# XieResearchGroup/Physics-aware-Multiplex-GNN

Measured on AMD Instinct MI355X. Metric: molecules/sec (QM9 dim=128 n_layer=6) at 1/2/4/8 GPU; scatter-add HBM GB/s vs peak, higher is better.
Workload: dtype f32; 1 GPU; QM9-schema synthetic radius-graph batches, PAMNet dim=128 n_layer=6, 128 molecules/GPU (BASELINE configs[1]), full training step fwd+bwd+allreduce+clip+Adam+EMA; global_batch=128, parallelism=dp1 (molecule-sharded, RCCL all-reduce of flat grad), nodes_per_batch=2286, global_edges=32888, local_edges=4316, triplets=6662, pairs=10978

## Files before the change

include/pamnet_hip.h:

```cpp
#ifndef PAMNET_HIP_H
#define PAMNET_HIP_H

#include <stdint.h>

#ifdef __cplusplus
extern "C" {
#endif

#define PAMNET_OK 0
#define PAMNET_EINVAL (-1)
#define PAMNET_ENULL (-2)
#define PAMNET_WEIGHT_IMAGES 2
#define PAMNET_CHAIN_PIECES 16

typedef void* pamnet_stream_t;

#define PAMNET_ABI_VERSION 18
int pamnet_abi_version(void);

int pamnet_segment_sum_f32(float* out, const float* init, const float* A, const int32_t* ia, const float* B,
                           const int32_t* ib, const int32_t* perm, const int32_t* ptr, int64_t rows, int64_t d,
                           pamnet_stream_t stream);

int pamnet_gather_mul_f32(float* out, const float* A, const int32_t* ia, const float* B, const int32_t* ib,
// ... 269 lines not shown
                         const int32_t* band_status, const uint8_t* climb, const double* k_b, double k, float* dneb,
                         double* seg, double* fpar, pamnet_stream_t stream);

int pamnet_vib_displace_f32(const float* pos0, const int32_t* gptr, const int32_t* fptr, const int32_t* free_idx, int64_t n,
                            int64_t n_graphs, int64_t pairs, int64_t t, double delta, float* pos_out, pamnet_stream_t stream);
int pamnet_vib_rows_f64(const float* dpos, const float* pos0, const float* masses, const int32_t* fptr, const int32_t* free_idx,
                        const int64_t* moff, int64_t n, int64_t n_graphs, int64_t pairs, int64_t t, double delta, double* h,
                        pamnet_stream_t stream);
int pamnet_sym_eig_f64(double* a, double* v, double* w, int32_t* status, int32_t* sweeps, const int64_t* moff,
                       const int64_t* dptr, int64_t n_mat, double tol, int32_t max_sweeps, pamnet_stream_t stream);

int pamnet_md_step_f32(float* pos, float* vel, const float* dpos, const float* mass, const uint8_t* fixed, const int32_t* gptr,
                       int64_t n, int64_t n_graphs, const int64_t* seed, int32_t* steps, int32_t* status, double* ke,
                       const double* dt_g, const double* kT_g, const double* gamma_g, double dt, double kT, double gamma,
                       int32_t kick_in, int32_t advance, pamnet_stream_t stream);
int pamnet_md_init_velocities_f32(float* vel, const float* mass, const uint8_t* fixed, const int32_t* gptr, int64_t n,
                                  int64_t n_graphs, const int64_t* seed, const double* kT_g, double kT, int32_t remove_com,
                                  int32_t rescale, double* ke, pamnet_stream_t stream);

int pamnet_md_npt_step_f32(float* pos, float* vel, const float* dpos, const float* dstrain, const float* mass,
                           const uint8_t* fixed, const int32_t* gptr, int64_t n, int64_t n_graphs, const float* cell0,
                           float* cell, double* eps, const uint8_t* cell_dof, const int64_t* seed, int32_t* steps,
                           int32_t* status, double* ke, double* pint, double* vol, const double* dt_g, const double* kT_g,
                           const double* gamma_g, const double* pressure_g, const double* rate_g, double dt, double kT,
                           double gamma, double pressure, double rate, int32_t kick_in, int32_t advance,
                           pamnet_stream_t stream);

int pamnet_fuse_pool_fwd_f32(const float* outs, const float* atts, int64_t n_layer, int64_t n, const float* sign,
                             const int32_t* gptr, int64_t n_graphs, int32_t mean, float* node_out, float* graph_out,
                             pamnet_stream_t stream);
int pamnet_fuse_pool_bwd_f32(const float* outs, const float* atts, int64_t n_layer, int64_t n, const float* sign,
                             const int32_t* node_graph, const int32_t* gptr, int32_t mean, const float* grad_graph,
                             float* grad_outs, float* grad_atts, pamnet_stream_t stream);

int pamnet_node_tail_fwd_f32(const float* x2, const float* res_x, int64_t n, const float* const* weights,
                             const float* const* biases, const float* w_out, const float* b_out, const float* w_att,
                             float* Z, float* R, float* x_out, float* out, float* att, const float* next_Wx1,
                             const float* next_bx1, const float* const* next_wp, int64_t next_ldwp, int64_t next_nblk,
                             float* next_Zx1, float* next_x1, float* next_P, int32_t packed, pamnet_stream_t stream);
int pamnet_node_tail_fwd_rider_f32(const float* x2, const float* res_x, int64_t n, const float* const* weights,
                                   const float* const* biases, const float* w_out, const float* b_out,
                                   const float* w_att, float* Z, float* R, float* x_out, const float* next_Wx1,
                                   const float* next_bx1, const float* const* next_wp, int64_t next_ldwp,
                                   int64_t next_nblk, float* next_Zx1, float* next_x1, float* next_P, const float* mlp_x,
                                   int64_t mlp_rows, int64_t mlp_tile0, int64_t mlp_ntiles, const float* const* mlp,
                                   float* const* mlp_out, int64_t rider_wgs, int32_t packed ,
                                   pamnet_stream_t stream);
int pamnet_node_heads_fwd_f32(int64_t n_layers, const float* const* x_out, const float* const* weights,
                              const float* const* biases, const float* const* w_out, const float* const* b_out,
                              const float* const* w_att, float* const* Z, float* const* out, float* const* att, int64_t n,
                              int32_t packed, pamnet_stream_t stream);
int pamnet_node_tail_bwd_f32(const float* d_xout, const float* d_out, const float* d_att, int64_t n,
                             const float* const* weights, const float* w_out, const float* w_att, const float* Z,
                             float* dZ, float* d_x2, float* d_resx, float* head_partial, float* d_wout, float* d_watt,
                             float* d_bout, int32_t packed, pamnet_stream_t stream);
int pamnet_node_heads_bwd_f32(int64_t n_layers, const float* const* d_out, const float* const* d_att,
                              const float* const* weights, const float* const* w_out, const float* const* w_att,
                              const float* const* Z, float* const* dZ3, float* const* g_head, float* const* head_partial,
                              int64_t n, int32_t packed, pamnet_stream_t stream);
int pamnet_node_tail_main_bwd_f32(const float* d_xout, const float* g_head, int64_t n, const float* const* weights,
                                  const float* Z, float* dZ, float* d_x2, float* d_resx, int32_t packed,
                                  pamnet_stream_t stream);
int pamnet_node_pre_tail_bwd_f32(const float* dP, const float* dx1_direct, const float* d_add, int64_t n,
                                 const float* Wx1, const float* const* wp, int64_t nblk, const float* Zx1, float* dZx1,
                                 const float* g_head, const float* const* weights, const float* Z, float* dZ,
                                 float* d_x2, float* d_resx, const void* rider ,
// ... 259 lines not shown
```

physics-aware-multiplex-gnn_amd/csrc/basis.hip:

```cpp
#include "common.h"
#include "basis_constants.h"

namespace {

__device__ __forceinline__ float envelope_f(float x) {
    if (!(x < 1.0f)) return 0.0f;
    const float x2 = x * x, x5 = x2 * x2 * x;
    return 1.0f / x + x5 * (-21.0f + x * (35.0f - 15.0f * x));
}

__device__ __forceinline__ double envelope_d(double x) {
    if (!(x < 1.0)) return 0.0;
    const double x2 = x * x, x5 = x2 * x2 * x;
    return 1.0 / x + x5 * (-21.0 + x * (35.0 - 15.0 * x));
}

constexpr int SERIES_TERMS = 28;
struct SeriesTab {
    double c[7][SERIES_TERMS + 1];
    double inv_dfact[7];
};
constexpr SeriesTab make_series() {
    SeriesTab t{};
    for (int l = 0; l < 7; ++l) {
        t.c[l][0] = 1.0;
        for (int k = 1; k <= SERIES_TERMS; ++k) t.c[l][k] = t.c[l][k - 1] * -0.5 / ((double)k * (double)(2 * l + 2 * k + 1));
        double d = 1.0;
        for (int m = 1; m <= l; ++m) d *= (double)(2 * m + 1);
        t.inv_dfact[l] = 1.0 / d;
    }
    return t;
}
__device__ __constant__ SeriesTab SBF_SERIES = make_series();
// ... 312 lines not shown
    const int lane = threadIdx.x & 63;
    if (q >= m) return;
    const double x = (double)(dist[q] * inv_cf);
    if (!(x < 1.0)) {
        if (lane == 0) ddist[q] = 0.0f;
        return;
    }
    double v = 0.0;
    if (lane < 42) {
        const int l = lane / 6;
        double acc = 0.0;
        for (int k = tt_ptr[q]; k < tt_ptr[q + 1]; ++k) {
            const int64_t t = tt_perm[k];
            const double ct = cos((double)angle[t]);
            double p0 = 1.0, p1 = ct;
            for (int j = 2; j <= l; ++j) {
                const double pj = ((double)(2 * j - 1) * ct * p1 - (double)(j - 1) * p0) / (double)j;
                p0 = p1;
                p1 = pj;
            }
            acc += (double)gsbf[t * 42 + lane] * PAMNET_YL0_PREF[l] * (l == 0 ? 1.0 : p1);
        }
        const double env = envelope_d(x), denv = envelope_dx_d(x);
        const double z = (double)PAMNET_SBF_ZEROS_F32[lane], u = z * x;
        const double jl = sph_jl(l, u);
        const double djl = (l == 0) ? -sph_jl(1, u) : sph_jl(l - 1, u) - (double)(l + 1) / u * jl;
        v = acc * PAMNET_SBF_NORM[lane] * (denv * jl + env * z * djl);
    }
#pragma unroll
    for (int o = 32; o >= 1; o >>= 1) v += __shfl_xor(v, o, 64);
    if (lane == 0) ddist[q] = (float)(v * inv_cutoff);
}

__device__ __forceinline__ float leaky02(float a) { return a > 0.f ? a : 0.2f * a; }

__global__ __launch_bounds__(256) void fuse_node_kernel(const float* __restrict__ outs, const float* __restrict__ atts,
                                                        int n_layer, int64_t n, const float* __restrict__ sign,
                                                        float* __restrict__ node_out) {
    const int64_t v = (int64_t)blockIdx.x * blockDim.x + threadIdx.x;
    if (v >= n) return;
    float acc = 0.f;
    for (int l = 0; l < n_layer; ++l) {
        const float ag = leaky02(atts[(int64_t)(2 * l) * n + v]), al = leaky02(atts[(int64_t)(2 * l + 1) * n + v]);
        const float mx = fmaxf(ag, al);
        const float eg = expf(ag - mx), el = expf(al - mx);
        const float inv = 1.0f / (eg + el);
        acc += (outs[(int64_t)(2 * l) * n + v] * eg + outs[(int64_t)(2 * l + 1) * n + v] * el) * inv;
    }
    node_out[v] = sign ? acc * sign[v] : acc;
}

__global__ __launch_bounds__(256) void pool_kernel(const float* __restrict__ node_out, const int32_t* __restrict__ gptr,
                                                   int64_t n_graphs, int mean, float* __restrict__ graph_out) {
    const int lane = threadIdx.x & 63;
    const int64_t g = ((int64_t)blockIdx.x * blockDim.x + threadIdx.x) >> 6;
    if (g >= n_graphs) return;
    const int beg = gptr[g], end = gptr[g + 1];
    float s0 = 0.f, s1 = 0.f, s2 = 0.f, s3 = 0.f;
    int v = beg + lane;
    for (; v + 192 < end; v += 256) {
        s0 += node_out[v];
        s1 += node_out[v + 64];
        s2 += node_out[v + 128];
        s3 += node_out[v + 192];
    }
    for (; v < end; v += 64) s0 += node_out[v];
    float s = (s0 + s1) + (s2 + s3);
#pragma unroll
    for (int o = 32; o >= 1; o >>= 1) s += __shfl_xor(s, o, 64);
    if (lane == 0) graph_out[g] = mean ? s / (float)max(end - beg, 1) : s;
}

__global__ __launch_bounds__(256) void fuse_pool_bwd_kernel(const float* __restrict__ outs,
                                                            const float* __restrict__ atts, int n_layer, int64_t n,
                                                            const float* __restrict__ sign,
                                                            const int32_t* __restrict__ node_graph,
                                                            const int32_t* __restrict__ gptr, int mean,
                                                            const float* __restrict__ grad_graph,
                                                            float* __restrict__ grad_outs,
                                                            float* __restrict__ grad_atts) {
    const int64_t v = (int64_t)blockIdx.x * blockDim.x + threadIdx.x;
    if (v >= n) return;
    const int g = node_graph[v];
    float gn = grad_graph[g];
    if (mean) gn /= (float)max(gptr[g + 1] - gptr[g], 1);
    if (sign) gn *= sign[v];
    for (int l = 0; l < n_layer; ++l) {
        const int64_t ig = (int64_t)(2 * l) * n + v, il = (int64_t)(2 * l + 1) * n + v;
        const float rg = atts[ig], rl = atts[il];
        const float ag = leaky02(rg), al = leaky02(rl);
        const float mx = fmaxf(ag, al);
        const float eg = expf(ag - mx), el = expf(al - mx);
        const float inv = 1.0f / (eg + el);
        const float wg = eg * inv, wl = el * inv;
        grad_outs[ig] = gn * wg;
        grad_outs[il] = gn * wl;
        const float da = gn * (outs[ig] - outs[il]) * wg * wl;
        grad_atts[ig] = da * (rg > 0.f ? 1.0f : 0.2f);
        grad_atts[il] = -da * (rl > 0.f ? 1.0f : 0.2f);
    }
}

inline unsigned blocks_for(int64_t n, int per = 256) { return (unsigned)(n > 0 ? ceil_div(n, per) : 1); }

}

extern "C" int pamnet_abi_version(void) { return PAMNET_ABI_VERSION; }

extern "C" int pamnet_rbf_fwd_f32(const float* dist, const float* freq, float cutoff, int64_t m, float* rbf,
                                  pamnet_stream_t stream) {
    if (m < 0 || !(cutoff > 0.f)) return PAMNET_EINVAL;
    if (m == 0) return PAMNET_OK;
    if (!dist || !freq || !rbf) return PAMNET_ENULL;
    hipLaunchKernelGGL(rbf_fwd_kernel, dim3(blocks_for(m * 16)), dim3(256), 0, as_stream(stream), dist, freq,
                       1.0f / cutoff, m, rbf);
    PAMNET_LAUNCH_CHECK();
    return PAMNET_OK;
}

extern "C" int pamnet_rbf_bwd_f32(const float* dist, const float* freq, float cutoff, int64_t m, const float* grad,
                                  float* dfreq, float* partial, pamnet_stream_t stream) {
    if (m < 0 || !(cutoff > 0.f)) return PAMNET_EINVAL;
    if (!dfreq || !partial || (m > 0 && (!dist || !freq || !grad))) return PAMNET_ENULL;
    hipStream_t st = as_stream(stream);
    int nblocks = (int)(m > 0 ? (ceil_div(m, 16) < 2048 ? ceil_div(m, 16) : 2048) : 0);
    if (nblocks > 0) {
        hipLaunchKernelGGL(rbf_bwd_partial_kernel, dim3(nblocks), dim3(256), 0, st, dist, freq, 1.0f / cutoff, m, grad,
                           partial);
        PAMNET_LAUNCH_CHECK();
    }
    hipLaunchKernelGGL(rbf_bwd_final_kernel, dim3(1), dim3(1024), 0, st, partial, nblocks, dfreq);
    PAMNET_LAUNCH_CHECK();
    return PAMNET_OK;
// ... 110 lines not shown

extern "C" int pamnet_fuse_pool_fwd_f32(const float* outs, const float* atts, int64_t n_layer, int64_t n,
                                        const float* sign, const int32_t* gptr, int64_t n_graphs, int32_t mean,
                                        float* node_out, float* graph_out, pamnet_stream_t stream) {
    if (n_layer <= 0 || n < 0 || n_graphs < 0) return PAMNET_EINVAL;
    if (n_graphs == 0) return PAMNET_OK;
    hipStream_t st = as_stream(stream);
    if (n == 0) {
        if (!graph_out) return PAMNET_ENULL;
        return (int)hipMemsetAsync(graph_out, 0, sizeof(float) * (size_t)n_graphs, st);
    }
    if (!outs || !atts || !gptr || !node_out || !graph_out) return PAMNET_ENULL;
    hipLaunchKernelGGL(fuse_node_kernel, dim3(blocks_for(n)), dim3(256), 0, st, outs, atts, (int)n_layer, n, sign,
                       node_out);
    PAMNET_LAUNCH_CHECK();
    hipLaunchKernelGGL(pool_kernel, dim3(blocks_for(n_graphs, 4)), dim3(256), 0, st, node_out, gptr, n_graphs,
                       (int)mean, graph_out);
    PAMNET_LAUNCH_CHECK();
    return PAMNET_OK;
}

extern "C" int pamnet_fuse_pool_bwd_f32(const float* outs, const float* atts, int64_t n_layer, int64_t n,
                                        const float* sign, const int32_t* node_graph, const int32_t* gptr,
                                        int32_t mean, const float* grad_graph, float* grad_outs, float* grad_atts,
                                        pamnet_stream_t stream) {
    if (n_layer <= 0 || n < 0) return PAMNET_EINVAL;
    if (n == 0) return PAMNET_OK;
    if (!outs || !atts || !node_graph || !gptr || !grad_graph || !grad_outs || !grad_atts) return PAMNET_ENULL;
    hipLaunchKernelGGL(fuse_pool_bwd_kernel, dim3(blocks_for(n)), dim3(256), 0, as_stream(stream), outs, atts,
                       (int)n_layer, n, sign, node_graph, gptr, (int)mean, grad_graph, grad_outs, grad_atts);
    PAMNET_LAUNCH_CHECK();
    return PAMNET_OK;
}
```

physics-aware-multiplex-gnn_amd/csrc/reduce.hip:

```cpp
#include "common.h"
#include "type_rows_core.h"

namespace {

constexpr int NORM_BLOCKS = 256;

__global__ __launch_bounds__(256) void sumsq_partials_kernel(const float4* __restrict__ g, int64_t n4,
                                                             double* __restrict__ partial) {
    __shared__ double red[256];
    float4 a0 = make_float4(0.f, 0.f, 0.f, 0.f), a1 = a0;
    const int64_t per = (n4 + gridDim.x - 1) / gridDim.x;
    const int64_t beg = blockIdx.x * per, end = beg + per < n4 ? beg + per : n4;
    int64_t i = beg + threadIdx.x;
    for (; i + 256 < end; i += 512) {
        const float4 u = g[i], v = g[i + 256];
        a0.x = fmaf(u.x, u.x, a0.x), a0.y = fmaf(u.y, u.y, a0.y), a0.z = fmaf(u.z, u.z, a0.z), a0.w = fmaf(u.w, u.w, a0.w);
        a1.x = fmaf(v.x, v.x, a1.x), a1.y = fmaf(v.y, v.y, a1.y), a1.z = fmaf(v.z, v.z, a1.z), a1.w = fmaf(v.w, v.w, a1.w);
    }
    if (i < end) {
        const float4 u = g[i];
        a0.x = fmaf(u.x, u.x, a0.x), a0.y = fmaf(u.y, u.y, a0.y), a0.z = fmaf(u.z, u.z, a0.z), a0.w = fmaf(u.w, u.w, a0.w);
    }
    red[threadIdx.x] = ((double)a0.x + (double)a0.y) + ((double)a0.z + (double)a0.w) + ((double)a1.x + (double)a1.y) +
                       ((double)a1.z + (double)a1.w);
    __syncthreads();
    for (int s = 128; s > 0; s >>= 1) {
        if ((int)threadIdx.x < s) red[threadIdx.x] += red[threadIdx.x + s];
        __syncthreads();
    }
    if (threadIdx.x == 0) partial[blockIdx.x] = red[0];
}

__global__ __launch_bounds__(256) void sumsq_partials_masked_kernel(const float4* __restrict__ g, int64_t n4,
// ... 22 lines not shown
    __syncthreads();
    for (int s = 128; s > 0; s >>= 1) {
        if ((int)threadIdx.x < s) red[threadIdx.x] += red[threadIdx.x + s];
        __syncthreads();
    }
    if (threadIdx.x == 0) partial[blockIdx.x] = red[0];
}

__global__ __launch_bounds__(256) void grad_accumulate_kernel(float4* __restrict__ acc, float4* __restrict__ g, int64_t n4) {
    const float4 zero = make_float4(0.f, 0.f, 0.f, 0.f);
    const int64_t stride = (int64_t)gridDim.x * 256;
    int64_t i = (int64_t)blockIdx.x * 256 + threadIdx.x;
    for (; i + stride < n4; i += 2 * stride) {
        float4 a0 = acc[i], a1 = acc[i + stride];
        const float4 g0 = g[i], g1 = g[i + stride];
        a0.x += g0.x, a0.y += g0.y, a0.z += g0.z, a0.w += g0.w;
        a1.x += g1.x, a1.y += g1.y, a1.z += g1.z, a1.w += g1.w;
        acc[i] = a0, acc[i + stride] = a1;
        g[i] = zero, g[i + stride] = zero;
    }
    if (i < n4) {
        float4 a0 = acc[i];
        const float4 g0 = g[i];
        a0.x += g0.x, a0.y += g0.y, a0.z += g0.z, a0.w += g0.w;
        acc[i] = a0;
        g[i] = zero;
    }
}

template <int KIND>
__global__ __launch_bounds__(256) void loss_kernel(const float* __restrict__ out, const float* __restrict__ y, int64_t n,
                                                   float grad_scale, float* __restrict__ loss, float* __restrict__ d_out) {
    __shared__ double red[256];
    double s = 0.0;
    const float gs = grad_scale / (float)n;
    for (int64_t i = threadIdx.x; i < n; i += 256) {
        const float d = out[i] - y[i];
        const float a = fabsf(d);
        float l, dl;
        if (KIND == 0) {
            l = a, dl = d > 0.f ? 1.f : (d < 0.f ? -1.f : 0.f);
        } else if (KIND == 1) {
            l = d * d, dl = 2.f * d;
        } else {
            l = a < 1.f ? 0.5f * d * d : a - 0.5f, dl = a < 1.f ? d : (d > 0.f ? 1.f : -1.f);
        }
        s += (double)l;
        if (d_out) d_out[i] = dl * gs;
    }
    red[threadIdx.x] = s;
    __syncthreads();
    for (int k = 128; k > 0; k >>= 1) {
        if ((int)threadIdx.x < k) red[threadIdx.x] += red[threadIdx.x + k];
        __syncthreads();
    }
    if (threadIdx.x == 0) loss[0] = (float)(red[0] / (double)n);
}

template <int KIND>
int loss_launch(const float* out, const float* y, int64_t n, float grad_scale, float* loss, float* d_out,
                pamnet_stream_t stream) {
    if (n < 1) return PAMNET_EINVAL;
    if (!out || !y || !loss) return PAMNET_ENULL;
    hipLaunchKernelGGL(loss_kernel<KIND>, dim3(1), dim3(256), 0, as_stream(stream), out, y, n, grad_scale, loss, d_out);
    PAMNET_LAUNCH_CHECK();
    return PAMNET_OK;
}

using type_rows::TYPE_BLOCKS;
using type_rows::TYPE_MAX;

__global__ __launch_bounds__(256) void type_rows_grad_kernel(const float4* __restrict__ g, const int32_t* __restrict__ idx,
                                                             int64_t n, int n_types, int d4, float4* __restrict__ partial) {
    __shared__ float4 red[256];
    type_rows::grad_body(g, idx, n, n_types, d4, partial, blockIdx.x, gridDim.x, red);
}

__global__ __launch_bounds__(256) void type_rows_finish_kernel(const float4* __restrict__ partial, int blocks, int cells,
                                                               float4* __restrict__ out) {
    type_rows::finish_body(partial, blocks, cells, out);
}

__global__ __launch_bounds__(256) void type_rows_grad_wide_kernel(const float4* __restrict__ g, const int32_t* __restrict__ idx,
                                                                  int64_t n, int n_types, int d4, uint32_t* __restrict__ masks,
                                                                  float4* __restrict__ partial) {
    __shared__ float4 red[256];
    __shared__ uint32_t seen[4];
    type_rows::grad_wide_body(g, idx, n, n_types, d4, masks, partial, blockIdx.x, gridDim.x, red, seen);
// ... 142 lines not shown
```

physics-aware-multiplex-gnn_amd/models.py:

```python
import math
import os

import torch
import torch.nn as nn
import torch.nn.functional as F

from pamnet_amd import fused, narrow, stack
from pamnet_amd import graph as G
from pamnet_amd import ops
from pamnet_amd.modules import MLP, BesselBasis, GlobalMP, LocalMP, mlp_apply


class Config(object):
    def __init__(self, dataset, dim, n_layer, cutoff_l, cutoff_g, flow='source_to_target'):
        self.dataset = dataset
        self.dim = dim
        self.n_layer = n_layer
        self.cutoff_l = cutoff_l
        self.cutoff_g = cutoff_g
        self.flow = flow


def _sph_jn(l, x):
    if x < l + 1.0:
# ... 164 lines not shown
    torch.set_rng_state(cpu)
    if dev is not None:
        for i, st in enumerate(dev):
            torch.cuda.set_rng_state(st, i)


def engine_width(dim):
    for w in ENGINE_WIDTHS:
        if dim <= w:
            return w
    return (int(dim) + 3) // 4 * 4


class _PAMNetBase(nn.Module):
    small = False
    max_num_neighbors = 1000

    def __init__(self, config, num_spherical=7, num_radial=6, envelope_exponent=5, _pad=True, num_atom_types=5,
                 max_atomic_number=None):
        super().__init__()
        self.dataset = config.dataset
        self.config_dim = int(config.dim)
        w = engine_width(self.config_dim) if _pad else None
        self.dim = w if w is not None else self.config_dim
        self.n_layer = config.n_layer
        self.cutoff_l = config.cutoff_l
        self.cutoff_g = config.cutoff_g
        self.flow = getattr(config, 'flow', 'source_to_target')
        if self.config_dim < 1:
            raise ValueError('dim must be positive')
        self.__dict__['_rng_at_ctor'] = _rng_snapshot() if (_pad and self.dim != self.config_dim) else None
        self._rna = self.dataset[:3].lower() == 'rna'
        self.__dict__['_pending_checks'] = []
        self.__dict__['_ctor'] = (config, num_spherical, num_radial, envelope_exponent)
        if isinstance(num_atom_types, bool) or not isinstance(num_atom_types, int) or not 1 <= num_atom_types <= ops.TYPE_MAX:
            raise ValueError('num_atom_types must be an integer in 1..%d (got %r)' % (ops.TYPE_MAX, num_atom_types))
        if num_atom_types != 5 and self.dataset != 'QM9':
            raise ValueError('num_atom_types applies to the QM9 schema only (PDBbind rows carry features, the RNA table has '
                             'its three types): dataset is %r' % (self.dataset,))
        if max_atomic_number is not None:
            zmax = ops.TYPE_ROWS_MAX - 1
            if (isinstance(max_atomic_number, bool) or not isinstance(max_atomic_number, int)
                    or not 1 <= max_atomic_number <= zmax):
                raise ValueError('max_atomic_number must be an integer in 1..%d (got %r)' % (zmax, max_atomic_number))
            if num_atom_types != 5:
                raise ValueError('max_atomic_number and num_atom_types are two ways to size the same table: give one '
                                 '(got max_atomic_number=%r with num_atom_types=%r)' % (max_atomic_number, num_atom_types))
            if self.dataset != 'QM9':
                raise ValueError('max_atomic_number applies to the QM9 schema only (PDBbind rows carry features, the RNA '
                                 'table has its three types): dataset is %r' % (self.dataset,))
            num_atom_types = max_atomic_number + 1
        self.max_atomic_number = max_atomic_number
        self.num_atom_types = num_atom_types

    def named_parameters(self, prefix='', recurse=True, remove_duplicate=True):
        if prefix != '' or not recurse or not remove_duplicate:
            yield from super().named_parameters(prefix, recurse, remove_duplicate)
            return
        flat = self._flat_view()
        if flat is not None:
            yield (FLAT_NAME, flat.param)
            return
        yield from self._real_named_parameters()

    def _real_named_parameters(self):
        cache = self.__dict__.get('_named_param_cache')
# ... 272 lines not shown
                return None
            layers.append((feats, None, None, None, False, False))
            params.append(self.init_linear.weight)
        else:
            if not ops.type_rows_supported(self.embeddings):
                return None
            col = x_raw if self.dataset == 'QM9' else (x_raw.unsqueeze(-1) if x_raw.dim() == 1 else x_raw)[:, -1]
            types = g.types if getattr(g, 'types', None) is not None else col.to(torch.int32).contiguous()
            params.append(self.embeddings)
        outs = fused.input_stage(fused.InputSpec(layers, types), params, tape=tape)
        return outs[3], outs[0], outs[1], outs[2]

    @staticmethod
    def _embed_fused(x, seq):
        return len(seq) == 1 and fused.embed_supported(x, seq[0][0])

    def _run_layers(self, x, e_l, e_g, e_sbf, g, tape=None):
        if stack.engine_supported(x, g):
            outs, atts, saved = stack.layer_stack(self.global_layer, self.local_layer, x, e_g, e_l, e_sbf, g, tape=tape,
                                                  checked=bool(self.__dict__.get('_params_checked')))
            self._x_layers = _LazyLayers(saved, g, self.n_layer, x.size(1))
            return outs, atts
        outs, atts = [], []
        self._x_layers = []
        for k in range(self.n_layer):
            x, o, a = self.global_layer[k](x, e_g, g)
            outs.append(o), atts.append(a), self._x_layers.append(x)
            x, o, a = self.local_layer[k](x, e_l, e_sbf, g)
            outs.append(o), atts.append(a), self._x_layers.append(x)
        return ops.stack_rows(outs), ops.stack_rows(atts)

    def _layers_and_pool(self, x, e_l, e_g, e_sbf, g, tape, mean):
        outs, atts = self._run_layers(x, e_l, e_g, e_sbf, g, tape)
        out, node_out = ops.fuse_pool(outs, atts, g, mean=mean, tape=tape)
        self._graph_cache, self._node_out = g, node_out
        return out if tape is not None else out.view(-1)

    def _positions_with_grad(self, data):
        if not torch.is_grad_enabled():
            return None
        if self.dataset == 'QM9':
            src = getattr(data, 'pos', None)
            if src is None or not src.requires_grad:
                return None
        else:
            x = data.x
            if not x.requires_grad or x.dim() != 2:
                return None
            src = x[:, :3]
        if not self.sbf.default:
            raise NotImplementedError('PAMNet: gradients with respect to the positions are implemented for the default basis '
                                      '(num_spherical=7, num_radial=6, envelope_exponent=5) only; this model has (%d, %d, %d)'
                                      % (self.sbf.num_spherical, self.sbf.num_radial, self.sbf.envelope_exponent))
        return src.to(torch.float32).contiguous()

    def _geometry_inputs(self, data, g):
        pos = self._positions_with_grad(data)
        strain = getattr(data, 'strain', None) if torch.is_grad_enabled() else None
        if strain is None or not strain.requires_grad:
            return None if pos is None else (pos, None)
        if not self.sbf.default:
            raise NotImplementedError('PAMNet: gradients with respect to the strain are implemented for the default basis '
                                      '(num_spherical=7, num_radial=6, envelope_exponent=5) only; this model has (%d, %d, %d)'
                                      % (self.sbf.num_spherical, self.sbf.num_radial, self.sbf.envelope_exponent))
        if not getattr(g, 'strain_checked', False):
            raise ValueError('`data.strain` was attached after model.prepare(data): attach it first (the graph built ahead of '
                             'time validates it), or call model(data) without prepare')
# ... 193 lines not shown
```

physics-aware-multiplex-gnn_amd/pamnet_amd/ops.py:

```python
import ctypes

import torch

from . import lib


def _c(t):
    return t if t.is_contiguous() else t.contiguous()


class _NoGradCtx(object):
    needs_input_grad = ()

    def save_for_backward(self, *tensors):
        pass

    def mark_non_differentiable(self, *tensors):
        pass

    def set_materialize_grads(self, value):
        pass


import os as _os

TAPE = _os.environ.get('PAMNET_TAPE', '1') != '0'
import threading as _threading

_tls = _threading.local()


def _tape_stack_of_thread():
    st = getattr(_tls, 'stack', None)
    if st is None:
        st = _tls.stack = []
    return st


def current_tape():
    st = getattr(_tls, 'stack', None)
    return st[-1] if st else None


class no_direct_writes(object):

    def __enter__(self):
        _tls.no_direct = getattr(_tls, 'no_direct', 0) + 1

    def __exit__(self, *exc):
        _tls.no_direct -= 1


def direct_allowed():
    return not getattr(_tls, 'no_direct', 0)


def apply(fn, *args, tape=None):
    tape = tape if tape is not None else current_tape()
    if tape is not None:
# ... 319 lines not shown
                     lib.ptr(ddist), lib.stream_of(g))
        return ddist, dfreq, None, None


class _FusePool(torch.autograd.Function):

    @staticmethod
    def forward(ctx, outs, atts, graph, mean):
        outs, atts = _c(outs), _c(atts)
        n_layer, n = outs.size(0) // 2, outs.size(1)
        node_out = torch.empty(n, dtype=outs.dtype, device=outs.device)
        gout = torch.empty(graph.n_graphs, dtype=outs.dtype, device=outs.device)
        lib.call('pamnet_fuse_pool_fwd_f32', lib.ptr(outs), lib.ptr(atts), n_layer, n, lib.ptr(graph.sign),
                 lib.ptr(graph.gptr), graph.n_graphs, 1 if mean else 0, lib.ptr(node_out), lib.ptr(gout),
                 lib.stream_of(outs))
        ctx.save_for_backward(outs, atts)
        ctx.graph, ctx.mean = graph, mean
        ctx.mark_non_differentiable(node_out)
        return gout, node_out

    @staticmethod
    def backward(ctx, g, _g_node):
        outs, atts = ctx.saved_tensors
        graph = ctx.graph
        g = _c(g)
        n_layer, n = outs.size(0) // 2, outs.size(1)
        go, ga = torch.empty_like(outs), torch.empty_like(atts)
        lib.call('pamnet_fuse_pool_bwd_f32', lib.ptr(outs), lib.ptr(atts), n_layer, n, lib.ptr(graph.sign),
                 lib.ptr(graph.node_graph), lib.ptr(graph.gptr), 1 if ctx.mean else 0, lib.ptr(g), lib.ptr(go),
                 lib.ptr(ga), lib.stream_of(g))
        return go, ga, None, None


def _dense_scratch(n, k, m, like):
    floats = ctypes.c_int64(0)
    lib.call('pamnet_dense_scratch_floats', n, k, m, ctypes.addressof(floats))
    return torch.empty(floats.value, dtype=torch.float32, device=like.device)


def _dense_fwd(x, w, b, act, keep_z):
    if x.dtype != torch.float32 or w.dtype != torch.float32:
        raise TypeError('pamnet dense kernels compute in float32: got %s x %s' % (x.dtype, w.dtype))
    n, k = x.shape
    m = w.size(0)
    y = torch.empty(n, m, dtype=x.dtype, device=x.device)
    z = torch.empty_like(y) if (act and keep_z) else None
    lib.call('pamnet_dense_fwd_f32', lib.ptr(x), k, lib.ptr(w), k, lib.ptr(b), n, k, m, 1 if act else 0, lib.ptr(z),
             lib.ptr(y), lib.stream_of(x))
    return y, z


def _dense_bwd(g, z, x, w, act, need_dx, need_dw, need_db):
    n, k = x.shape
    m = g.size(1)
    dx = torch.empty(n, k, dtype=g.dtype, device=g.device) if need_dx else None
    need_dw = need_dw or need_db
    dw = torch.empty(m, k, dtype=g.dtype, device=g.device) if need_dw else None
    db = torch.empty(m, dtype=g.dtype, device=g.device) if need_db else None
    scratch = _dense_scratch(n, k, m, g) if need_dw else None
    lib.call('pamnet_dense_bwd_f32', lib.ptr(g), lib.ptr(z), lib.ptr(x), k, lib.ptr(w), k, n, k, m, 1 if act else 0,
             lib.ptr(dx), lib.ptr(dw), lib.ptr(db), lib.ptr(scratch), lib.stream_of(g))
    return dx, dw, db


def embed_input_grad(x, g, kind, sets, act=True):
    x = _c(x)
# ... 110 lines not shown
```

physics-aware-multiplex-gnn_amd/pamnet_amd/train.py:

```python
import math
import re

import torch
import torch.distributed as dist
import torch.nn.functional as F


_LAYER_RE = re.compile(r'^(?:global_layer|local_layer)\.(\d+)\.')


def _layer_of(name):
    m = _LAYER_RE.match(name)
    return int(m.group(1)) if m else None


class FlatParams(object):

    def __init__(self, module, direct=True):
        named = [(n, p) for n, p in getattr(module, '_real_named_parameters', module.named_parameters)() if p.requires_grad]
        rank = lambda n: (1, 0) if _layer_of(n) is None else (0, -_layer_of(n))
        named.sort(key=lambda np_: rank(np_[0]))
        self.params = [p for _, p in named]
        self.names = [n for n, _ in named]
        dev, dt = self.params[0].device, self.params[0].dtype
# ... 303 lines not shown
            st = self.opt.state.get(self._p, {})
            if 'exp_avg' in st:
                m.copy_(st['exp_avg']), v.copy_(st['exp_avg_sq'])
            return m, v
        for o, k, view in self._views:
            st = self.opt.state.get(view, {})
            if 'exp_avg' in st:
                m[o:o + k].copy_(st['exp_avg']), v[o:o + k].copy_(st['exp_avg_sq'])
        return m, v

    def accumulated_grad(self):
        return (self.fp.grad if self.acc is None else self.acc).clone()

    def _accumulate(self):
        if self.fp.flat.is_cuda:
            from . import lib
            lib.call('pamnet_grad_accumulate_f32', lib.ptr(self.acc), lib.ptr(self.fp.grad), self.fp.grad.numel(),
                     lib.stream_of(self.fp.grad))
        else:
            self.acc.add_(self.fp.grad)
            self.fp.grad.zero_()
        self._grad_clean = True

    def forward_backward(self, data, global_graphs=None):
        if not self._grad_clean:
            self.fp.zero_grad()
        self._grad_clean = False
        if self._stack_ctx is not None:
            self._stack_ctx.recorded = False
        if self._pack:
            self.fp.release_grads()
        plan = self._stack_plan_of_model()
        self._before = (plan, -1 if plan is None else plan.table_calls)
        out = self.model(data)
        try:
            self._check_ownership()
        except RuntimeError:
            del out
            if self._pack:
                self.fp.pack_grads()
            self._grad_clean = True
            raise
        split = self.world_size > 1 or self.accumulate > 1
        if split and global_graphs is None:
            global_graphs = out.numel() * self.world_size * self.accumulate
        scale = float(out.numel()) / float(global_graphs) if split else 1.0
        if out.is_cuda and out.dtype == torch.float32:
            from . import ops
            loss, d_out = ops.loss_with_grad(self.loss_kind, out, data.y, scale)
            if not ops.backward_whole(out, d_out):
                out.backward(d_out)
        else:
            loss = {'l1': F.l1_loss, 'mse': F.mse_loss, 'smooth_l1': F.smooth_l1_loss}[self.loss_kind](out, data.y)
            (loss * scale).backward()
        if self._pack:
            self.fp.pack_grads()
        return loss

    def _stack_plan_of_model(self):
        return getattr(getattr(self.model, 'global_layer', None), '__dict__', {}).get('_pamnet_plan')

    def _check_ownership(self):
        model = self.model
        ep = getattr(model, '__dict__', {}).get('_param_epoch')
        if ep is None:
            return
        plan = self._stack_plan_of_model()
        if plan is not None and (plan is not self._before[0] or plan.table_calls == self._before[1]):
            plan.param_tables()
        pkey = None if plan is None else plan._pkey
        if ep == self._seen_epoch and plan is self._seen_plan and pkey is self._seen_pkey and self._loose is not None \
                and all(p.data_ptr() == a for p, a in self._loose):
            return
        msg = self.fp.mismatch(model)
        if msg is not None:
            raise RuntimeError('Trainer: %s -- the optimiser would update a buffer the model does not read. Build a new '
                               'Trainer on the edited model (load_state_dict without assign=True copies in place and needs '
                               'none).' % msg)
        inside = set() if plan is None else set(id(p) for p in plan.flat)
        self._loose = [(p, p.data_ptr()) for p in self.fp.params if id(p) not in inside]
        self._seen_epoch, self._seen_plan, self._seen_pkey = ep, plan, pkey
# ... 386 lines not shown
```

Baseline: 70560 molecules/s.

## Defer readout and fuse pooling, loss and readout backward into fewer kernels

During training the model's final fuse-and-pool readout is deferred to a custom autograd node. The trainer then calls a single native entry that fuses node attention fusion with per-graph pooling in one kernel and computes the loss, its gradient and the readout backward in one further kernel. This removes separate launches for node fuse, pool, loss and the pool backward, plus one intermediate grad_graph round trip. In exchange it adds cross-module plumbing between the tape, model and trainer, and a planner heuristic chooses between the fused and the two-pass pooling.

```diff
diff --git a/include/pamnet_hip.h b/include/pamnet_hip.h
--- a/include/pamnet_hip.h
+++ b/include/pamnet_hip.h
@@ -325,6 +325,11 @@
 int pamnet_fuse_pool_bwd_f32(const float* outs, const float* atts, int64_t n_layer, int64_t n, const float* sign,
                              const int32_t* node_graph, const int32_t* gptr, int32_t mean, const float* grad_graph,
                              float* grad_outs, float* grad_atts, pamnet_stream_t stream);
+
+int pamnet_readout_loss_f32(const float* outs, const float* atts, int64_t n_layer, int64_t n, const float* sign,
+                            const int32_t* node_graph, const int32_t* gptr, int64_t n_graphs, int32_t mean, const float* y,
+                            int32_t loss_kind, float grad_scale, int32_t form, float* node_out, float* graph_out, float* loss,
+                            float* grad_graph, float* grad_outs, float* grad_atts, pamnet_stream_t stream);
 
 int pamnet_node_tail_fwd_f32(const float* x2, const float* res_x, int64_t n, const float* const* weights,
                              const float* const* biases, const float* w_out, const float* b_out, const float* w_att,
diff --git a/physics-aware-multiplex-gnn_amd/csrc/basis.hip b/physics-aware-multiplex-gnn_amd/csrc/basis.hip
--- a/physics-aware-multiplex-gnn_amd/csrc/basis.hip
+++ b/physics-aware-multiplex-gnn_amd/csrc/basis.hip
@@ -1,4 +1,5 @@
 #include "common.h"
+#include "readout_core.h"
 #include "basis_constants.h"
 
 namespace {
@@ -377,30 +378,16 @@
     if (lane == 0) ddist[q] = (float)(v * inv_cutoff);
 }
 
-__device__ __forceinline__ float leaky02(float a) { return a > 0.f ? a : 0.2f * a; }
-
 __global__ __launch_bounds__(256) void fuse_node_kernel(const float* __restrict__ outs, const float* __restrict__ atts,
                                                         int n_layer, int64_t n, const float* __restrict__ sign,
                                                         float* __restrict__ node_out) {
     const int64_t v = (int64_t)blockIdx.x * blockDim.x + threadIdx.x;
     if (v >= n) return;
-    float acc = 0.f;
-    for (int l = 0; l < n_layer; ++l) {
-        const float ag = leaky02(atts[(int64_t)(2 * l) * n + v]), al = leaky02(atts[(int64_t)(2 * l + 1) * n + v]);
-        const float mx = fmaxf(ag, al);
-        const float eg = expf(ag - mx), el = expf(al - mx);
-        const float inv = 1.0f / (eg + el);
-        acc += (outs[(int64_t)(2 * l) * n + v] * eg + outs[(int64_t)(2 * l + 1) * n + v] * el) * inv;
-    }
-    node_out[v] = sign ? acc * sign[v] : acc;
-}
-
-__global__ __launch_bounds__(256) void pool_kernel(const float* __restrict__ node_out, const int32_t* __restrict__ gptr,
-                                                   int64_t n_graphs, int mean, float* __restrict__ graph_out) {
-    const int lane = threadIdx.x & 63;
-    const int64_t g = ((int64_t)blockIdx.x * blockDim.x + threadIdx.x) >> 6;
-    if (g >= n_graphs) return;
-    const int beg = gptr[g], end = gptr[g + 1];
+    node_out[v] = readout::fuse_node(outs, atts, n_layer, n, sign, v);
+}
+
+template <class Nodes>
+__device__ __forceinline__ float pool_wave(const Nodes& node_out, int beg, int end, int lane) {
     float s0 = 0.f, s1 = 0.f, s2 = 0.f, s3 = 0.f;
     int v = beg + lane;
     for (; v + 192 < end; v += 256) {
@@ -413,7 +400,44 @@
     float s = (s0 + s1) + (s2 + s3);
 #pragma unroll
     for (int o = 32; o >= 1; o >>= 1) s += __shfl_xor(s, o, 64);
-    if (lane == 0) graph_out[g] = mean ? s / (float)max(end - beg, 1) : s;
+    return s;
+}
+
+__global__ __launch_bounds__(256) void pool_kernel(const float* __restrict__ node_out, const int32_t* __restrict__ gptr,
+                                                   int64_t n_graphs, int mean, float* __restrict__ graph_out) {
+    const int lane = threadIdx.x & 63;
+    const int64_t g = ((int64_t)blockIdx.x * blockDim.x + threadIdx.x) >> 6;
+    if (g >= n_graphs) return;
+    const int beg = gptr[g], end = gptr[g + 1];
+    const float s = pool_wave(node_out, beg, end, lane);
+    if (lane == 0) graph_out[g] = readout::pool_value(s, beg, end, mean);
+}
+
+struct FusedNodes {
+    const float* __restrict__ outs;
+    const float* __restrict__ atts;
+    int n_layer;
+    int64_t n;
+    const float* __restrict__ sign;
+    float* __restrict__ store;
+    __device__ __forceinline__ float operator[](int v) const {
+        const float o = readout::fuse_node(outs, atts, n_layer, n, sign, v);
+        if (store) store[v] = o;
+        return o;
+    }
+};
+
+__global__ __launch_bounds__(256) void fuse_pool_kernel(const float* __restrict__ outs, const float* __restrict__ atts,
+                                                        int n_layer, int64_t n, const float* __restrict__ sign,
+                                                        const int32_t* __restrict__ gptr, int64_t n_graphs, int mean,
+                                                        float* __restrict__ node_out, float* __restrict__ graph_out) {
+    const int lane = threadIdx.x & 63;
+    const int64_t g = ((int64_t)blockIdx.x * blockDim.x + threadIdx.x) >> 6;
+    if (g >= n_graphs) return;
+    const int beg = gptr[g], end = gptr[g + 1];
+    const FusedNodes nodes = {outs, atts, n_layer, n, sign, node_out};
+    const float s = pool_wave(nodes, beg, end, lane);
+    if (lane == 0) graph_out[g] = readout::pool_value(s, beg, end, mean);
 }
 
 __global__ __launch_bounds__(256) void fuse_pool_bwd_kernel(const float* __restrict__ outs,
@@ -427,23 +451,33 @@
     const int64_t v = (int64_t)blockIdx.x * blockDim.x + threadIdx.x;
     if (v >= n) return;
     const int g = node_graph[v];
-    float gn = grad_graph[g];
-    if (mean) gn /= (float)max(gptr[g + 1] - gptr[g], 1);
-    if (sign) gn *= sign[v];
-    for (int l = 0; l < n_layer; ++l) {
-        const int64_t ig = (int64_t)(2 * l) * n + v, il = (int64_t)(2 * l + 1) * n + v;
-        const float rg = atts[ig], rl = atts[il];
-        const float ag = leaky02(rg), al = leaky02(rl);
-        const float mx = fmaxf(ag, al);
-        const float eg = expf(ag - mx), el = expf(al - mx);
-        const float inv = 1.0f / (eg + el);
-        const float wg = eg * inv, wl = el * inv;
-        grad_outs[ig] = gn * wg;
-        grad_outs[il] = gn * wl;
-        const float da = gn * (outs[ig] - outs[il]) * wg * wl;
-        grad_atts[ig] = da * (rg > 0.f ? 1.0f : 0.2f);
-        grad_atts[il] = -da * (rl > 0.f ? 1.0f : 0.2f);
-    }
+    readout::fuse_node_bwd(outs, atts, n_layer, n, sign, gptr[g + 1] - gptr[g], mean, grad_graph[g], v, grad_outs, grad_atts);
+}
+
+template <int KIND>
+__global__ __launch_bounds__(256) void loss_fuse_pool_bwd_kernel(const float* __restrict__ outs, const float* __restrict__ atts,
+                                                                 int n_layer, int64_t n, const float* __restrict__ sign,
+                                                                 const int32_t* __restrict__ node_graph,
+                                                                 const int32_t* __restrict__ gptr, int64_t n_graphs, int mean,
+                                                                 const float* __restrict__ graph_out,
+                                                                 const float* __restrict__ y, float grad_scale,
+                                                                 float* __restrict__ loss, float* __restrict__ grad_graph,
+                                                                 float* __restrict__ grad_outs, float* __restrict__ grad_atts) {
+    const float gs = grad_scale / (float)n_graphs;
+    if (blockIdx.x == gridDim.x - 1) {
+        __shared__ double red[256];
+        red[threadIdx.x] = readout::loss_partial<KIND>(graph_out, y, n_graphs, gs, grad_graph, threadIdx.x);
+        __syncthreads();
+        readout::loss_tree(red, threadIdx.x);
+        if (threadIdx.x == 0) loss[0] = (float)(red[0] / (double)n_graphs);
+        return;
+    }
+    const int64_t v = (int64_t)blockIdx.x * blockDim.x + threadIdx.x;
+    if (v >= n) return;
+    const int g = node_graph[v];
+    float l, dl;
+    readout::loss_term<KIND>(graph_out[g] - y[g], l, dl);
+    readout::fuse_node_bwd(outs, atts, n_layer, n, sign, gptr[g + 1] - gptr[g], mean, dl * gs, v, grad_outs, grad_atts);
 }
 
 inline unsigned blocks_for(int64_t n, int per = 256) { return (unsigned)(n > 0 ? ceil_div(n, per) : 1); }
@@ -620,3 +654,61 @@
     PAMNET_LAUNCH_CHECK();
     return PAMNET_OK;
 }
+
+namespace {
+
+constexpr int64_t READOUT_WAVE_ROWS = 64 * 2 * 6;
+
+inline bool plan_readout_fused_pool(int64_t n, int64_t n_graphs, int64_t n_layer) {
+    return n * 2 * n_layer <= READOUT_WAVE_ROWS * n_graphs;
+}
+
+template <int KIND>
+void loss_bwd_launch(const float* outs, const float* atts, int n_layer, int64_t n, const float* sign, const int32_t* node_graph,
+                     const int32_t* gptr, int64_t n_graphs, int mean, const float* graph_out, const float* y, float grad_scale,
+                     float* loss, float* grad_graph, float* grad_outs, float* grad_atts, hipStream_t st) {
+    hipLaunchKernelGGL(loss_fuse_pool_bwd_kernel<KIND>, dim3(blocks_for(n) + 1), dim3(256), 0, st, outs, atts, n_layer, n,
+                       sign, node_graph, gptr, n_graphs, mean, graph_out, y, grad_scale, loss, grad_graph, grad_outs,
+                       grad_atts);
+}
+
+}
+
+extern "C" int pamnet_readout_loss_f32(const float* outs, const float* atts, int64_t n_layer, int64_t n, const float* sign,
+                                       const int32_t* node_graph, const int32_t* gptr, int64_t n_graphs, int32_t mean,
+                                       const float* y, int32_t loss_kind, float grad_scale, int32_t form, float* node_out,
+                                       float* graph_out, float* loss, float* grad_graph, float* grad_outs, float* grad_atts,
+                                       pamnet_stream_t stream) {
+    if (n_layer <= 0 || n < 1 || n_graphs < 1 || loss_kind < 0 || loss_kind > 2 || form < 0 || form > 3) return PAMNET_EINVAL;
+    if (!outs || !atts || !node_graph || !gptr || !y || !graph_out || !loss || !grad_outs || !grad_atts) return PAMNET_ENULL;
+    if (form == 2 && !grad_graph) return PAMNET_ENULL;
+    hipStream_t st = as_stream(stream);
+    if (form == 1 || (form == 0 && plan_readout_fused_pool(n, n_graphs, n_layer))) {
+        hipLaunchKernelGGL(fuse_pool_kernel, dim3(blocks_for(n_graphs, 4)), dim3(256), 0, st, outs, atts, (int)n_layer, n, sign,
+                           gptr, n_graphs, (int)mean, node_out, graph_out);
+        PAMNET_LAUNCH_CHECK();
+    } else {
+        if (!node_out) return PAMNET_ENULL;
+        const int rc = pamnet_fuse_pool_fwd_f32(outs, atts, n_layer, n, sign, gptr, n_graphs, mean, node_out, graph_out, stream);
+        if (rc) return rc;
+    }
+    if (form == 2) {
+        const int rc = loss_kind == 0   ? pamnet_l1_loss_f32(graph_out, y, n_graphs, grad_scale, loss, grad_graph, stream)
+                       : loss_kind == 1 ? pamnet_mse_loss_f32(graph_out, y, n_graphs, grad_scale, loss, grad_graph, stream)
+                                        : pamnet_smooth_l1_loss_f32(graph_out, y, n_graphs, grad_scale, loss, grad_graph, stream);
+        if (rc) return rc;
+        return pamnet_fuse_pool_bwd_f32(outs, atts, n_layer, n, sign, node_graph, gptr, mean, grad_graph, grad_outs, grad_atts,
+                                        stream);
+    }
+    if (loss_kind == 0)
+        loss_bwd_launch<0>(outs, atts, (int)n_layer, n, sign, node_graph, gptr, n_graphs, (int)mean, graph_out, y, grad_scale,
+                           loss, grad_graph, grad_outs, grad_atts, st);
+    else if (loss_kind == 1)
+        loss_bwd_launch<1>(outs, atts, (int)n_layer, n, sign, node_graph, gptr, n_graphs, (int)mean, graph_out, y, grad_scale,
+                           loss, grad_graph, grad_outs, grad_atts, st);
+    else
+        loss_bwd_launch<2>(outs, atts, (int)n_layer, n, sign, node_graph, gptr, n_graphs, (int)mean, graph_out, y, grad_scale,
+                           loss, grad_graph, grad_outs, grad_atts, st);
+    PAMNET_LAUNCH_CHECK();
+    return PAMNET_OK;
+}
diff --git a/physics-aware-multiplex-gnn_amd/csrc/readout_core.h b/physics-aware-multiplex-gnn_amd/csrc/readout_core.h
--- /dev/null
+++ b/physics-aware-multiplex-gnn_amd/csrc/readout_core.h
@@ -0,0 +1,81 @@
+#pragma once
+#include "common.h"
+
+namespace readout {
+
+__device__ __forceinline__ float leaky02(float a) { return a > 0.f ? a : 0.2f * a; }
+
+__device__ __forceinline__ float fuse_node(const float* __restrict__ outs, const float* __restrict__ atts, int n_layer,
+                                           int64_t n, const float* __restrict__ sign, int64_t v) {
+    float acc = 0.f;
+#pragma unroll 6
+    for (int l = 0; l < n_layer; ++l) {
+        const float ag = leaky02(atts[(int64_t)(2 * l) * n + v]), al = leaky02(atts[(int64_t)(2 * l + 1) * n + v]);
+        const float mx = fmaxf(ag, al);
+        const float eg = expf(ag - mx), el = expf(al - mx);
+        const float inv = 1.0f / (eg + el);
+        acc += (outs[(int64_t)(2 * l) * n + v] * eg + outs[(int64_t)(2 * l + 1) * n + v] * el) * inv;
+    }
+    return sign ? acc * sign[v] : acc;
+}
+
+__device__ __forceinline__ float pool_value(float s, int beg, int end, int mean) {
+    return mean ? s / (float)max(end - beg, 1) : s;
+}
+
+template <int KIND>
+__device__ __forceinline__ void loss_term(float d, float& l, float& dl) {
+    const float a = fabsf(d);
+    if (KIND == 0) {
+        l = a, dl = d > 0.f ? 1.f : (d < 0.f ? -1.f : 0.f);
+    } else if (KIND == 1) {
+        l = d * d, dl = 2.f * d;
+    } else {
+        l = a < 1.f ? 0.5f * d * d : a - 0.5f, dl = a < 1.f ? d : (d > 0.f ? 1.f : -1.f);
+    }
+}
+
+template <int KIND>
+__device__ __forceinline__ double loss_partial(const float* __restrict__ out, const float* __restrict__ y, int64_t n, float gs,
+                                               float* __restrict__ d_out, int tid) {
+    double s = 0.0;
+    for (int64_t i = tid; i < n; i += 256) {
+        const float d = out[i] - y[i];
+        float l, dl;
+        loss_term<KIND>(d, l, dl);
+        s += (double)l;
+        if (d_out) d_out[i] = dl * gs;
+    }
+    return s;
+}
+
+__device__ __forceinline__ void loss_tree(double* red, int tid) {
+    for (int k = 128; k > 0; k >>= 1) {
+        if (tid < k) red[tid] += red[tid + k];
+        __syncthreads();
+    }
+}
+
+__device__ __forceinline__ void fuse_node_bwd(const float* __restrict__ outs, const float* __restrict__ atts, int n_layer,
+                                              int64_t n, const float* __restrict__ sign, int graph_nodes, int mean, float gn,
+                                              int64_t v, float* __restrict__ grad_outs, float* __restrict__ grad_atts) {
+    if (mean) gn /= (float)max(graph_nodes, 1);
+    if (sign) gn *= sign[v];
+#pragma unroll 6
+    for (int l = 0; l < n_layer; ++l) {
+        const int64_t ig = (int64_t)(2 * l) * n + v, il = (int64_t)(2 * l + 1) * n + v;
+        const float rg = atts[ig], rl = atts[il];
+        const float ag = leaky02(rg), al = leaky02(rl);
+        const float mx = fmaxf(ag, al);
+        const float eg = expf(ag - mx), el = expf(al - mx);
+        const float inv = 1.0f / (eg + el);
+        const float wg = eg * inv, wl = el * inv;
+        grad_outs[ig] = gn * wg;
+        grad_outs[il] = gn * wl;
+        const float da = gn * (outs[ig] - outs[il]) * wg * wl;
+        grad_atts[ig] = da * (rg > 0.f ? 1.0f : 0.2f);
+        grad_atts[il] = -da * (rl > 0.f ? 1.0f : 0.2f);
+    }
+}
+
+}
diff --git a/physics-aware-multiplex-gnn_amd/csrc/reduce.hip b/physics-aware-multiplex-gnn_amd/csrc/reduce.hip
--- a/physics-aware-multiplex-gnn_amd/csrc/reduce.hip
+++ b/physics-aware-multiplex-gnn_amd/csrc/reduce.hip
@@ -1,4 +1,5 @@
 #include "common.h"
+#include "readout_core.h"
 #include "type_rows_core.h"
 
 namespace {
@@ -87,28 +88,9 @@
 __global__ __launch_bounds__(256) void loss_kernel(const float* __restrict__ out, const float* __restrict__ y, int64_t n,
                                                    float grad_scale, float* __restrict__ loss, float* __restrict__ d_out) {
     __shared__ double red[256];
-    double s = 0.0;
-    const float gs = grad_scale / (float)n;
-    for (int64_t i = threadIdx.x; i < n; i += 256) {
-        const float d = out[i] - y[i];
-        const float a = fabsf(d);
-        float l, dl;
-        if (KIND == 0) {
-            l = a, dl = d > 0.f ? 1.f : (d < 0.f ? -1.f : 0.f);
-        } else if (KIND == 1) {
-            l = d * d, dl = 2.f * d;
-        } else {
-            l = a < 1.f ? 0.5f * d * d : a - 0.5f, dl = a < 1.f ? d : (d > 0.f ? 1.f : -1.f);
-        }
-        s += (double)l;
-        if (d_out) d_out[i] = dl * gs;
-    }
-    red[threadIdx.x] = s;
+    red[threadIdx.x] = readout::loss_partial<KIND>(out, y, n, grad_scale / (float)n, d_out, threadIdx.x);
     __syncthreads();
-    for (int k = 128; k > 0; k >>= 1) {
-        if ((int)threadIdx.x < k) red[threadIdx.x] += red[threadIdx.x + k];
-        __syncthreads();
-    }
+    readout::loss_tree(red, threadIdx.x);
     if (threadIdx.x == 0) loss[0] = (float)(red[0] / (double)n);
 }
 
diff --git a/physics-aware-multiplex-gnn_amd/models.py b/physics-aware-multiplex-gnn_amd/models.py
--- a/physics-aware-multiplex-gnn_amd/models.py
+++ b/physics-aware-multiplex-gnn_amd/models.py
@@ -220,6 +220,7 @@
         self.__dict__['_rng_at_ctor'] = _rng_snapshot() if (_pad and self.dim != self.config_dim) else None
         self._rna = self.dataset[:3].lower() == 'rna'
         self.__dict__['_pending_checks'] = []
+        self.__dict__['_defer_readout'] = False
         self.__dict__['_ctor'] = (config, num_spherical, num_radial, envelope_exponent)
         if isinstance(num_atom_types, bool) or not isinstance(num_atom_types, int) or not 1 <= num_atom_types <= ops.TYPE_MAX:
             raise ValueError('num_atom_types must be an integer in 1..%d (got %r)' % (ops.TYPE_MAX, num_atom_types))
@@ -558,7 +559,10 @@
 
     def _layers_and_pool(self, x, e_l, e_g, e_sbf, g, tape, mean):
         outs, atts = self._run_layers(x, e_l, e_g, e_sbf, g, tape)
-        out, node_out = ops.fuse_pool(outs, atts, g, mean=mean, tape=tape)
+        if self.__dict__.get('_defer_readout') and ops.readout_deferrable(outs, g, tape):
+            out, node_out = ops.fuse_pool_deferred(outs, atts, g, mean, tape)
+        else:
+            out, node_out = ops.fuse_pool(outs, atts, g, mean=mean, tape=tape)
         self._graph_cache, self._node_out = g, node_out
         return out if tape is not None else out.view(-1)
 
diff --git a/physics-aware-multiplex-gnn_amd/pamnet_amd/ops.py b/physics-aware-multiplex-gnn_amd/pamnet_amd/ops.py
--- a/physics-aware-multiplex-gnn_amd/pamnet_amd/ops.py
+++ b/physics-aware-multiplex-gnn_amd/pamnet_amd/ops.py
@@ -25,6 +25,7 @@
 import os as _os
 
 TAPE = _os.environ.get('PAMNET_TAPE', '1') != '0'
+READOUT_FUSED = _os.environ.get('PAMNET_READOUT_FUSED', '1') != '0'
 import threading as _threading
 
 _tls = _threading.local()
@@ -410,6 +411,68 @@
         return go, ga, None, None
 
 
+class _FusePoolDeferred(torch.autograd.Function):
+
+    @staticmethod
+    def forward(ctx, outs, atts, graph, mean):
+        outs, atts = _c(outs), _c(atts)
+        node_out = torch.empty(outs.size(1), dtype=outs.dtype, device=outs.device)
+        gout = torch.empty(graph.n_graphs, dtype=outs.dtype, device=outs.device)
+        ctx.save_for_backward(outs, atts)
+        ctx.graph, ctx.mean, ctx.node_out, ctx.gout, ctx.grads = graph, mean, node_out, gout, None
+        return gout, node_out
+
+    @staticmethod
+    def backward(ctx, g, _g_node):
+        if ctx.grads is None:
+            raise RuntimeError('the readout of this forward was left to ops.readout_loss(), which has not run')
+        grads, ctx.grads = ctx.grads, None
+        return grads[0], grads[1], None, None
+
+
+def readout_deferrable(outs, graph, tape):
+    return READOUT_FUSED and tape is not None and outs.is_cuda and outs.dtype == torch.float32 and outs.size(1) > 0 \
+        and graph.n_graphs > 0
+
+
+def fuse_pool_deferred(outs, atts, graph, mean, tape):
+    out = tape.call(_FusePoolDeferred, outs, atts, graph, mean)
+    tape.readout = tape.nodes[-1][1]
+    return out
+
+
+def pending_readout(out):
+    tape = getattr(out.grad_fn, 'tape', None)
+    ctx = getattr(tape, 'readout', None)
+    return ctx if ctx is not None and ctx.gout.data_ptr() == out.data_ptr() else None
+
+
+def readout_loss(kind, out, y, grad_scale=1.0):
+    ctx = pending_readout(out)
+    if kind not in LOSS_ENTRIES:
+        raise ValueError("loss must be one of 'l1', 'mse', 'smooth_l1' (got %r)" % (kind,))
+    if y.numel() != out.numel():
+        raise ValueError('%s loss: target has %d elements, the model output %d' % (kind, y.numel(), out.numel()))
+    if y.device != out.device or y.dtype != torch.float32 or y.shape != out.shape:
+        y = y.to(device=out.device, dtype=torch.float32).reshape(out.shape)
+    y = _c(y)
+    outs, atts = ctx.saved_tensors
+    graph = ctx.graph
+    n_layer, n = outs.size(0) // 2, outs.size(1)
+    loss = torch.empty(1, dtype=torch.float32, device=out.device)
+    gg = torch.empty_like(ctx.gout)
+    go, ga = torch.empty_like(outs), torch.empty_like(atts)
+    lib.call('pamnet_readout_loss_f32', lib.ptr(outs), lib.ptr(atts), n_layer, n, lib.ptr(graph.sign),
+             lib.ptr(graph.node_graph), lib.ptr(graph.gptr), graph.n_graphs, 1 if ctx.mean else 0, lib.ptr(y),
+             ('l1', 'mse', 'smooth_l1').index(kind), float(grad_scale), 0, lib.ptr(ctx.node_out), lib.ptr(ctx.gout),
+             lib.ptr(loss), lib.ptr(gg), lib.ptr(go), lib.ptr(ga), lib.stream_of(outs))
+    ctx.grads = (go, ga)
+    out.grad_fn.tape.readout = None
+    if not backward_whole(out, gg):
+        out.backward(gg)
+    return loss[0]
+
+
 def _dense_scratch(n, k, m, like):
     floats = ctypes.c_int64(0)
     lib.call('pamnet_dense_scratch_floats', n, k, m, ctypes.addressof(floats))
diff --git a/physics-aware-multiplex-gnn_amd/pamnet_amd/train.py b/physics-aware-multiplex-gnn_amd/pamnet_amd/train.py
--- a/physics-aware-multiplex-gnn_amd/pamnet_amd/train.py
+++ b/physics-aware-multiplex-gnn_amd/pamnet_amd/train.py
@@ -359,7 +359,14 @@
             self.fp.release_grads()
         plan = self._stack_plan_of_model()
         self._before = (plan, -1 if plan is None else plan.table_calls)
-        out = self.model(data)
+        defer = getattr(self.model, '__dict__', {}).get('_defer_readout') is False
+        if defer:
+            self.model.__dict__['_defer_readout'] = True
+        try:
+            out = self.model(data)
+        finally:
+            if defer:
+                self.model.__dict__['_defer_readout'] = False
         try:
             self._check_ownership()
         except RuntimeError:
@@ -374,6 +381,11 @@
         scale = float(out.numel()) / float(global_graphs) if split else 1.0
         if out.is_cuda and out.dtype == torch.float32:
             from . import ops
+            if ops.pending_readout(out) is not None:
+                loss = ops.readout_loss(self.loss_kind, out, data.y, scale)
+                if self._pack:
+                    self.fp.pack_grads()
+                return loss
             loss, d_out = ops.loss_with_grad(self.loss_kind, out, data.y, scale)
             if not ops.backward_whole(out, d_out):
                 out.backward(d_out)
```

After: 70720 molecules/s (median of 5 runs). About the same (+0.2%).
